# pangenome/sweepga

Measured on AMD Instinct MI355X. Metric: PAF mappings/sec through plane-sweep+scaffold filter, 1/2/4/8 MI355X, higher is better.
Workload: dtype u32 coordinates, f64 scores; 1 GPU; BASELINE.json configs[3] (synthetic 100 M mappings across 10 k (q,t) groups, 100-genome pangenome shape; S-pan in SURVEY.md 8d): 100000000 mappings per GPU over 9900 genome-pair groups (100 single-chromosome genomes), pipeline=default; flags=(defaults), mappings_per_gpu=100000000, groups_per_gpu=9900

## Files before the change

sweepga_amd/csrc/swg_chain_table.hip:

```cpp
#include "swg_scaffold_internal.h"

namespace swg_scaf {
namespace {

__global__ __launch_bounds__(EW) void seg_compose_kernel(uint64_t m, const uint32_t* __restrict__ s_gidx,
                                                         const uint32_t* __restrict__ v, int complement,
                                                         uint64_t* __restrict__ out) {
  uint64_t p = (uint64_t)blockIdx.x * EW + threadIdx.x;
  if (p < m) out[p] = ((uint64_t)s_gidx[p] << 32) | (complement ? 0xffffffffu - v[p] : v[p]);
}
__global__ __launch_bounds__(EW) void group_first_from_scan_kernel(uint64_t m, const uint32_t* __restrict__ head_flag,
                                                                   const uint64_t* __restrict__ run_max,
                                                                   uint32_t* __restrict__ group_first) {
  uint64_t p = (uint64_t)blockIdx.x * EW + threadIdx.x;
  if (p >= m) return;
  if (p + 1 == m || head_flag[p + 1]) {
    const uint64_t v = run_max[p];
    group_first[(uint32_t)(v >> 32)] = 0xffffffffu - (uint32_t)v;
  }
}

constexpr int HEAD_SPAN = 1024;
__global__ __launch_bounds__(EW) void head_init_kernel(uint64_t m, const uint32_t* __restrict__ pred,
                                                       uint32_t* __restrict__ hd, const uint8_t* __restrict__ only,
// ... 212 lines not shown
        if (*slot > vmin) atomicMin(slot, vmin);
      }
    } else {
#pragma unroll
      for (int u = 0; u < U; ++u)
        if (live[u]) {
          uint32_t* slot = pair_slot(table, (uint32_t)(L[u] >> 32), (uint32_t)L[u]);
          if (*slot > (uint32_t)(i0 + u)) atomicMin(slot, (uint32_t)(i0 + u));
        }
    }
  }
}

__global__ __launch_bounds__(EW) void genome_pair_first_groups_kernel(uint32_t n_groups, const uint32_t* __restrict__ group_begin,
                                                                      const uint32_t* __restrict__ s_idx,
                                                                      const uint32_t* __restrict__ group_first,
                                                                      const uint32_t* __restrict__ q_id,
                                                                      const uint32_t* __restrict__ t_id,
                                                                      const uint32_t* __restrict__ seq_genome, PairTable table) {
  uint32_t g = blockIdx.x * EW + threadIdx.x;
  if (g >= n_groups) return;
  const uint32_t i = s_idx[group_begin[g]];
  atomicMin(pair_slot(table, seq_genome[q_id[i]], seq_genome[t_id[i]]), group_first[g]);
}

__device__ __forceinline__ uint32_t heads_before(const uint32_t* __restrict__ ch_head, uint32_t nc, uint32_t p) {
  uint32_t l = 0, r = nc;
  while (l < r) {
    const uint32_t mid = l + ((r - l) >> 1);
    if (ch_head[mid] < p)
      l = mid + 1;
    else
      r = mid;
  }
  return l;
}
__global__ __launch_bounds__(EW) void group_keys_kernel(uint32_t n_groups, const uint32_t* __restrict__ group_begin,
                                                        uint32_t m, const uint32_t* __restrict__ ch_head, uint32_t nc,
                                                        const uint32_t* __restrict__ s_idx,
                                                        const uint32_t* __restrict__ group_first,
                                                        const uint32_t* __restrict__ q_id,
                                                        const uint32_t* __restrict__ t_id,
                                                        const uint32_t* __restrict__ seq_genome, bool pair_major,
                                                        PairTable gp_first, int idx_bits,
                                                        uint64_t* __restrict__ g_key, uint32_t* __restrict__ g_val,
                                                        uint32_t* __restrict__ g_first_chain,
                                                        uint32_t* __restrict__ g_nchains) {
  uint32_t g = blockIdx.x * EW + threadIdx.x;
  if (g >= n_groups) return;
  const uint32_t b = group_begin[g];
  const uint32_t first = heads_before(ch_head, nc, b);
  const uint32_t next = (g + 1 < n_groups) ? heads_before(ch_head, nc, group_begin[g + 1]) : nc;
  (void)m;
  g_first_chain[g] = first;
  g_nchains[g] = next - first;
  const uint32_t i = s_idx[b];
  uint64_t hi = 0;
  if (pair_major) hi = pair_get(gp_first, seq_genome[q_id[i]], seq_genome[t_id[i]]);
  g_key[g] = (hi << idx_bits) | group_first[g];
  g_val[g] = g;
}
__global__ __launch_bounds__(EW) void group_sizes_sorted_kernel(uint32_t n_groups, const uint32_t* __restrict__ g_sorted,
                                                                const uint32_t* __restrict__ g_nchains,
                                                                uint32_t* __restrict__ sizes) {
  uint32_t r = blockIdx.x * EW + threadIdx.x;
  if (r < n_groups) sizes[r] = g_nchains[g_sorted[r]];
}
__global__ __launch_bounds__(EW) void group_base_kernel(uint32_t n_groups, const uint32_t* __restrict__ g_sorted,
                                                        const uint32_t* __restrict__ base_sorted,
                                                        uint32_t* __restrict__ g_base) {
  uint32_t r = blockIdx.x * EW + threadIdx.x;
  if (r < n_groups) g_base[g_sorted[r]] = base_sorted[r];
}
__global__ __launch_bounds__(EW) void chain_place_kernel(uint64_t nc, const uint32_t* __restrict__ ch_head,
                                                         const uint32_t* __restrict__ s_gidx,
                                                         const uint32_t* __restrict__ g_first_chain,
                                                         const uint32_t* __restrict__ g_base, uint32_t* __restrict__ order) {
  uint64_t c = (uint64_t)blockIdx.x * EW + threadIdx.x;
  if (c >= nc) return;
  const uint32_t g = s_gidx[ch_head[c]];
  order[g_base[g] + ((uint32_t)c - g_first_chain[g])] = (uint32_t)c;
}

__global__ __launch_bounds__(EW) void chain_ok_kernel(uint64_t m, const uint32_t* __restrict__ is_head,
                                                      const uint32_t* __restrict__ s_qs, const uint32_t* __restrict__ h_qe,
                                                      const uint32_t* __restrict__ h_ts, const uint32_t* __restrict__ h_te,
                                                      const unsigned long long* __restrict__ h_sm,
                                                      const unsigned long long* __restrict__ h_sb,
                                                      const uint64_t* __restrict__ s_grp, uint64_t min_len,
                                                      double min_ident, uint8_t* __restrict__ ok_head,
                                                      HeadRec* __restrict__ rec, const uint8_t* __restrict__ only,
                                                      const uint8_t* __restrict__ span) {
  const uint64_t n_span = (m + HEAD_SPAN - 1) / HEAD_SPAN;
  for (uint64_t sp = blockIdx.x; sp < n_span; sp += gridDim.x) {
    if (span && !span[sp]) continue;
    for (int k = threadIdx.x; k < HEAD_SPAN; k += EW) {
      const uint64_t p = sp * HEAD_SPAN + k;
      if (p >= m) break;
      if (only && !only[p]) continue;
      bool ok = false;
      if (is_head[p] != 0) {
        const uint64_t total_length = (uint64_t)h_qe[p] - (uint64_t)s_qs[p];
        ok = total_length >= min_len;
        if (ok) {
          const double wid = chain_weighted_identity(total_length, h_sm[p], h_sb[p]);
          ok = wid >= min_ident;
          if (ok) {
            HeadRec hr;
            hr.qs = s_qs[p];
            hr.qe = h_qe[p];
            hr.ts = h_ts[p];
            hr.te = h_te[p];
            hr.wid = wid;
            hr.grp = s_grp[p];
            rec[p] = hr;
          }
        }
      }
      ok_head[p] = ok ? 1 : 0;
    }
  }
}

constexpr int LABEL_CAP = (int)(WALK_CHUNK + BIG_UNIT);
constexpr int LABEL_FAST = (int)LABEL_FAST_ELEMS;
constexpr int LABEL_NT = 512;
static_assert(LABEL_FAST * (2 + 2 + 3 * 4) >= LABEL_CAP * 2, "the two layouts share one LDS buffer");
template <int NT, bool MB, bool RANKED>
__global__ __launch_bounds__(NT, RANKED ? 8 : 1) void chain_label_kernel(uint32_t n_chunks, const SpecBlock* __restrict__ chunks,
                                                         const uint32_t* __restrict__ pred,
                                                         const uint32_t* __restrict__ s_qs, const uint32_t* __restrict__ s_qe,
                                                         const uint32_t* __restrict__ s_ts, const uint32_t* __restrict__ s_te,
                                                         const uint32_t* __restrict__ s_m, const uint32_t* __restrict__ s_b,
                                                         const uint64_t* __restrict__ s_grp,
                                                         uint64_t min_len, double min_ident, uint32_t* __restrict__ hd,
                                                         uint8_t* __restrict__ ok_head, HeadRec* __restrict__ rec,
                                                         unsigned long long* __restrict__ n_heads,
                                                         const uint32_t* __restrict__ n_chunks_dev = nullptr, LabelRanked R = LabelRanked{}) {
  if (n_chunks_dev) n_chunks = min(n_chunks, *n_chunks_dev);
  __shared__ uint32_t lds[LABEL_FAST * (MB ? 6 : 4)];
  uint16_t* succ = reinterpret_cast<uint16_t*>(lds);
  uint16_t* l_hd = succ + LABEL_FAST;
  uint32_t* l_qe = lds + LABEL_FAST;
  uint32_t* l_ts = l_qe + LABEL_FAST;
  uint32_t* l_te = l_ts + LABEL_FAST;
  uint32_t* l_m = MB ? l_te + LABEL_FAST : nullptr;
  uint32_t* l_b = MB ? l_m + LABEL_FAST : nullptr;
  __shared__ uint64_t ws64[RANKED ? NT / 64 : 1];
  if (!MB) s_m = s_b = nullptr;
  constexpr uint16_t NO = 0xffffu;
  uint32_t heads = 0;
  for (uint32_t c = blockIdx.x; c < n_chunks; c += gridDim.x) {
    const uint32_t b = chunks[c].bb, e = chunks[c].be;
    uint32_t len = e > b ? e - b : 0;
    if (len >= (uint32_t)LABEL_CAP) len = 0;
    __syncthreads();
    for (uint32_t k = threadIdx.x; k < len; k += NT) succ[k] = NO;
    __syncthreads();
    if (len <= (uint32_t)LABEL_FAST) {
      constexpr int U = LABEL_FAST / NT;
      static_assert(LABEL_FAST % NT == 0, "whole rounds");
      uint32_t r_pr[U], r_qe[U], r_ts[U], r_te[U], r_m[U], r_b[U], r_qs[U];
#pragma unroll
      for (int u = 0; u < U; ++u) {
        const uint32_t k = (uint32_t)u * NT + threadIdx.x;
        const uint32_t p = b + (k < len ? k : 0u);
        r_pr[u] = pred[p];
        r_qe[u] = s_qe[p];
        r_ts[u] = s_ts[p];
        r_te[u] = s_te[p];
        r_m[u] = s_m ? s_m[p] : 0u;
        r_b[u] = s_m ? s_b[p] : 0u;
        r_qs[u] = s_qs[p];
      }
#pragma unroll
      for (int u = 0; u < U; ++u) {
        const uint32_t k = (uint32_t)u * NT + threadIdx.x;
        if (k < len) {
          if (r_pr[u] != NONE) succ[r_pr[u] - b] = (uint16_t)k;
          l_hd[k] = r_pr[u] != NONE ? NO : (uint16_t)k;
          l_qe[k] = r_qe[u];
          l_ts[k] = r_ts[u];
          l_te[k] = r_te[u];
          if constexpr (MB) {
            l_m[k] = r_m[u];
            l_b[k] = r_b[u];
          }
        }
      }
      __syncthreads();
      const uint32_t pad = RANKED ? chunks[c].pad : 0u;
      const bool rkd = RANKED && (pad & CHUNK_RANKED) != 0u;
      uint32_t pass = 0;
#pragma unroll
      for (int u = 0; u < U; ++u) {
        const uint32_t k = (uint32_t)u * NT + threadIdx.x;
        if (k >= len) continue;
        const uint32_t p = b + k;
        if (r_pr[u] != NONE) {
          if (!rkd) ok_head[p] = 0;
          continue;
        }
        ++heads;
        uint32_t qe = r_qe[u], ts = r_ts[u], te = r_te[u];
        uint64_t sm = r_m[u], sb = r_b[u];
        for (uint16_t nx = succ[k]; nx != NO; nx = succ[nx]) {
          const uint32_t a = l_qe[nx], t0 = l_ts[nx], t1 = l_te[nx];
          l_hd[nx] = (uint16_t)k;
          qe = a > qe ? a : qe;
          ts = t0 < ts ? t0 : ts;
          te = t1 > te ? t1 : te;
          if constexpr (MB) {
            sm += l_m[nx];
            sb += l_b[nx];
          }
        }
        const uint32_t qs0 = r_qs[u];
        const uint64_t total_length = (uint64_t)qe - (uint64_t)qs0;
        bool ok = total_length >= min_len;
        if (ok) {
          const double wid = chain_weighted_identity(total_length, sm, sb);
          ok = wid >= min_ident;
          if (ok && !rkd) {
            HeadRec hr;
            hr.qs = qs0;
            hr.qe = qe;
            hr.ts = ts;
            hr.te = te;
            hr.wid = wid;
            hr.grp = s_grp ? s_grp[p] : 0ull;
            rec[p] = hr;
          }
        }
        if (rkd) {
          if (ok) {
            pass |= 1u << u;
            l_qe[k] = qe;
            l_ts[k] = ts;
            l_te[k] = qs0;
            if (!(qs0 < qe && ts < te)) atomicOr(R.flags, R.fallback_bit);
          } else {
            succ[k] = NO;
          }
          continue;
        }
        ok_head[p] = ok ? (uint8_t)(s_grp ? 1u : 1u | (qs0 < qe ? 2u : 0u) | (ts < te ? 4u : 0u)) : (uint8_t)0;
      }
      if constexpr (RANKED) {
        if (rkd) {
          uint64_t packed = 0;
#pragma unroll
          for (int u = 0; u < U; ++u) packed |= (uint64_t)((pass >> u) & 1u) << (16 * u);
          static_assert(U <= 4 && NT < 65536, "the rows' counters share a 64-bit word");
          uint64_t inc = packed;
          const int lane = threadIdx.x & 63, w = threadIdx.x >> 6;
#pragma unroll
          for (int d = 1; d < 64; d <<= 1) {
            const uint64_t t = __shfl_up(inc, d, 64);
            if (lane >= d) inc += t;
          }
          if (lane == 63) ws64[w] = inc;
          __syncthreads();
          uint64_t off = 0, tot = 0;
#pragma unroll
          for (int j = 0; j < NT / 64; ++j) {
            const uint64_t x = ws64[j];
            off += j < w ? x : 0ull;
            tot += x;
          }
          const uint64_t ex = off + inc - packed;
          uint32_t row_base = 0;
#pragma unroll
          for (int u = 0; u < U; ++u) {
            const uint32_t k = (uint32_t)u * NT + threadIdx.x;
            if ((pass >> u) & 1u) {
              const uint32_t r = row_base + (uint32_t)((ex >> (16 * u)) & 0xffffu);
              succ[k] = (uint16_t)r;
              if ((pad & 1u) == 0u) {
                R.t_qs[b + r] = l_te[k];
                R.t_qe[b + r] = l_qe[k];
                reinterpret_cast<uint32_t*>(rec + b)[r] = l_ts[k];
              }
            }
            row_base += (uint32_t)((tot >> (16 * u)) & 0xffffu);
          }
          if (threadIdx.x == 0) R.chunk_pass[c] = row_base;
          __syncthreads();
          for (uint32_t k = threadIdx.x; k < len; k += NT) {
            const uint16_t r = succ[l_hd[k]];
            hd[b + k] = r == NO ? NONE : (uint32_t)r;
          }
          continue;
        }
      }
      __syncthreads();
      for (uint32_t k = threadIdx.x; k < len; k += NT) hd[b + k] = b + l_hd[k];
      continue;
    }
    constexpr int LB = 2048 / NT;
    for (uint32_t k0 = 0; k0 < len; k0 += NT * LB) {
      uint32_t pr[LB];
#pragma unroll
      for (int u = 0; u < LB; ++u) {
        const uint32_t k = k0 + (uint32_t)u * NT + threadIdx.x;
        pr[u] = pred[b + (k < len ? k : 0u)];
      }
#pragma unroll
      for (int u = 0; u < LB; ++u) {
        const uint32_t k = k0 + (uint32_t)u * NT + threadIdx.x;
        if (k < len && pr[u] != NONE) succ[pr[u] - b] = (uint16_t)k;
      }
    }
    __syncthreads();
    for (uint32_t k0 = 0; k0 < len; k0 += NT * LB) {
      uint32_t pr[LB], v_qs[LB], v_qe[LB], v_ts[LB], v_te[LB], v_m[LB], v_b[LB];
#pragma unroll
      for (int u = 0; u < LB; ++u) {
        const uint32_t k = k0 + (uint32_t)u * NT + threadIdx.x;
        const uint32_t p = b + (k < len ? k : 0u);
        pr[u] = pred[p];
        v_qs[u] = s_qs[p];
        v_qe[u] = s_qe[p];
        v_ts[u] = s_ts[p];
        v_te[u] = s_te[p];
        v_m[u] = s_m ? s_m[p] : 0u;
        v_b[u] = s_m ? s_b[p] : 0u;
      }
#pragma unroll
      for (int u = 0; u < LB; ++u) {
        const uint32_t k = k0 + (uint32_t)u * NT + threadIdx.x;
        if (k >= len) continue;
        const uint32_t p = b + k;
        if (pr[u] != NONE) {
          ok_head[p] = 0;
          continue;
        }
        ++heads;
        hd[p] = p;
        uint32_t qe = v_qe[u], ts = v_ts[u], te = v_te[u];
        uint64_t sm = v_m[u], sb = v_b[u];
        for (uint16_t nx = succ[k]; nx != NO;) {
          const uint32_t q = b + nx;
          const uint16_t nn = succ[nx];
          const uint32_t a = s_qe[q], t0 = s_ts[q], t1 = s_te[q], mm = s_m ? s_m[q] : 0u, bb = s_m ? s_b[q] : 0u;
          hd[q] = p;
          qe = a > qe ? a : qe;
          ts = t0 < ts ? t0 : ts;
          te = t1 > te ? t1 : te;
          sm += mm;
          sb += bb;
          nx = nn;
        }
        const uint32_t qs0 = v_qs[u];
        const uint64_t total_length = (uint64_t)qe - (uint64_t)qs0;
        bool ok = total_length >= min_len;
        if (ok) {
          const double wid = chain_weighted_identity(total_length, sm, sb);
          ok = wid >= min_ident;
          if (ok) {
            HeadRec hr;
            hr.qs = qs0;
            hr.qe = qe;
            hr.ts = ts;
            hr.te = te;
            hr.wid = wid;
            hr.grp = s_grp ? s_grp[p] : 0ull;
            rec[p] = hr;
          }
        }
        ok_head[p] = ok ? (uint8_t)(s_grp ? 1u : 1u | (qs0 < qe ? 2u : 0u) | (ts < te ? 4u : 0u)) : (uint8_t)0;
      }
    }
  }
#pragma unroll
  for (int o = 32; o > 0; o >>= 1) heads += __shfl_down(heads, o, 64);
  __syncthreads();
  if ((threadIdx.x & 63) == 0) lds[threadIdx.x >> 6] = heads;
  __syncthreads();
  if (threadIdx.x == 0) {
    uint32_t all = 0;
    for (int w = 0; w < NT / 64; ++w) all += lds[w];
    if (all) atomicAdd(n_heads, (unsigned long long)all);
  }
}
__global__ __launch_bounds__(1024) void chain_label_long_kernel(uint32_t cap_long, const uint32_t* __restrict__ n_long_dev,
                                                                const uint32_t* __restrict__ long_list,
                                                                const SpecBlock* __restrict__ chunks, const uint32_t* __restrict__ pred,
                                                                const uint32_t* __restrict__ s_qs, const uint32_t* __restrict__ s_qe,
                                                                const uint32_t* __restrict__ s_ts, const uint32_t* __restrict__ s_te,
                                                                const uint32_t* __restrict__ s_m, const uint32_t* __restrict__ s_b,
                                                                uint64_t min_len, double min_ident, uint32_t* hd,
                                                                uint8_t* __restrict__ ok_head, HeadRec* rec,
                                                                unsigned long long* __restrict__ n_heads) {
// ... 341 lines not shown
```

sweepga_amd/csrc/swg_pair.hip:

```cpp
#include <cmath>
#include <type_traits>

#include "swg_scaffold_internal.h"

namespace swg_scaf {
namespace {

constexpr uint32_t PAIR_CELL = WALK_CHUNK;
constexpr uint32_t PAIR_S_MAX = 1024, PAIR_M_MAX = 4096, PAIR_L_MAX = 32768, PAIR_XL_MAX = uint32_t(1) << 18;
constexpr uint32_t PAIR_XL_CELLS = PAIR_XL_MAX / PAIR_CELL;
constexpr uint32_t PAIR_HASH_MAX = 65536;
constexpr uint32_t PAIR_MX_MAX = 16384, PAIR_MX_CUT_DEFAULT = 8192;
constexpr uint32_t ORDER_BIN_L = 128;
constexpr uint32_t ORDERED = 0x80000000u;
constexpr uint32_t PF_NOT_GROUPED = 1, PF_RUN_OVERFLOW = 2, PF_TOO_LONG = 4, PF_FALLBACK = 8;

struct PairRun {
  uint32_t a, n;
};
struct PairInfo {
  uint32_t m;
  uint32_t m_plus;
  uint32_t M;
  uint32_t first_alive;
// ... 1536 lines not shown
  uint8_t* status;
  uint32_t* chain;
  int scaffolds_only;
  uint64_t gap;
  uint64_t max_dev;
  uint64_t rescue_d;
  uint64_t max_s2;
  const uint8_t* kept_in;
  const uint32_t* chain_base;
  const uint32_t* np;
  const SpecBlock* chunks;
  uint32_t cap_chunks;
  const uint32_t* chunk_pass;
  uint32_t* rec_w;
  unsigned long long* ranked_stat;
  uint32_t* fin;
  uint32_t* anum;
  uint32_t* n_out_pair;
  PairCounters* C;
};
constexpr uint32_t NEVER = 0xfffffffeu;

struct PairChainArgs {
  const PairRun* runs;
  const uint32_t* list;
  const uint32_t* list_xl;
  uint32_t n_xl;
  const PairInfo* info;
  const uint8_t* ok_head;
  const HeadRec* rec;
  uint32_t *T_qs, *T_qe, *T_ts, *T_te;
  double* T_wid;
  uint64_t* T_seg;
  uint32_t *chain_base, *np;
  uint32_t *cnt, *has, *stretch;
  PairRun* T_runs;
  unsigned long long* totals;
  const PairCounters* C;
};
template <int NT, int PHASE>
__global__ __launch_bounds__(NT) void pair_chains_kernel(PairChainArgs A) {
  constexpr int U = 4;
  __shared__ uint32_t ws[NT / 64 + 1];
  __shared__ uint64_t ws64[NT / 64 + 1];
  __shared__ uint32_t sh_base;
  const int tid = threadIdx.x;
  if (A.C->flags & PF_FALLBACK) return;
  const uint32_t rk = blockIdx.x < A.n_xl ? A.list_xl[blockIdx.x] : A.list[blockIdx.x - A.n_xl];
  const PairRun run = A.runs[rk];
  const PairInfo pi = A.info[rk];
  const uint32_t a = run.a, m = pi.m, m_plus = pi.m_plus;
  if (PHASE == 0) {
    uint32_t c0 = 0, c1 = 0, mx = 0;
    for (uint32_t p0 = 0; p0 < m; p0 += NT * U) {
      uint8_t ok[U];
#pragma unroll
      for (int u = 0; u < U; ++u) {
        const uint32_t p = p0 + (uint32_t)u * NT + (uint32_t)tid;
        ok[u] = p < m ? A.ok_head[a + p] : (uint8_t)0;
      }
#pragma unroll
      for (int u = 0; u < U; ++u) {
        const uint32_t p = p0 + (uint32_t)u * NT + (uint32_t)tid;
        if (ok[u]) {
          const HeadRec hr = A.rec[a + p];
          if (p < m_plus) ++c0; else ++c1;
          const uint32_t e = hr.qe > hr.te ? hr.qe : hr.te;
          mx = e > mx ? e : mx;
        }
      }
    }
    const uint32_t nP = block_sum<NT>(c0, ws), nM = block_sum<NT>(c1, ws);
#pragma unroll
    for (int o = 32; o > 0; o >>= 1) {
      const uint32_t t = __shfl_xor(mx, o, 64);
      mx = t > mx ? t : mx;
    }
    if ((tid & 63) == 0 && (unsigned long long)mx > __hip_atomic_load(&A.totals[1], __ATOMIC_RELAXED, __HIP_MEMORY_SCOPE_AGENT))
      atomicMax(&A.totals[1], (unsigned long long)mx);
    if (tid == 0) {
      A.np[2 * rk] = nP;
      A.np[2 * rk + 1] = nM;
      A.cnt[rk] = nP + nM;
      A.has[rk] = nP + nM ? 1u : 0u;
    }
    return;
  }
  const uint32_t nP = A.np[2 * rk], nM = A.np[2 * rk + 1];
  if (nP + nM == 0) return;
  const uint32_t cb = A.chain_base[rk];
  if (tid == 0) {
    PairRun tr;
    tr.a = cb;
    tr.n = nP + nM;
    A.T_runs[A.stretch[rk]] = tr;
  }
  (void)sh_base;
  const bool plus_first = pi.first_mem[0] < pi.first_mem[1];
  uint32_t before = 0;
  for (uint32_t p0 = 0; p0 < m; p0 += NT * U) {
    uint8_t ok[U];
    uint64_t packed = 0;
#pragma unroll
    for (int u = 0; u < U; ++u) {
      const uint32_t p = p0 + (uint32_t)u * NT + (uint32_t)tid;
      ok[u] = p < m ? A.ok_head[a + p] : (uint8_t)0;
      packed |= (uint64_t)(ok[u] ? 1u : 0u) << (16 * u);
    }
    uint64_t inc = packed;
    const int lane = tid & 63, w = tid >> 6;
#pragma unroll
    for (int d = 1; d < 64; d <<= 1) {
      const uint64_t t = __shfl_up(inc, d, 64);
      if (lane >= d) inc += t;
    }
    uint64_t off = 0, tot = 0;
    if (NT == 64) {
      tot = __shfl(inc, 63, 64);
    } else {
      __syncthreads();
      if (lane == 63) ws64[w] = inc;
      __syncthreads();
#pragma unroll
      for (int k = 0; k < NT / 64; ++k) {
        const uint64_t x = ws64[k];
        off += k < w ? x : 0ull;
        tot += x;
      }
    }
    const uint64_t ex = off + inc - packed;
    uint32_t row_base = before;
#pragma unroll
    for (int u = 0; u < U; ++u) {
      const uint32_t p = p0 + (uint32_t)u * NT + (uint32_t)tid;
      if (ok[u]) {
        const uint32_t c_pos = row_base + (uint32_t)((ex >> (16 * u)) & 0xffffu);
        const uint32_t c_all = plus_first ? c_pos : (p >= m_plus ? c_pos - nP : c_pos + nM);
        const HeadRec hr = A.rec[a + p];
        const uint32_t c = cb + c_all;
        A.T_qs[c] = hr.qs;
        A.T_qe[c] = hr.qe;
        A.T_ts[c] = hr.ts;
        A.T_te[c] = hr.te;
        A.T_wid[c] = hr.wid;
        A.T_seg[c] = rk;
      }
      row_base += (uint32_t)((tot >> (16 * u)) & 0xffffu);
    }
    before = row_base;
  }
}

template <int NT, int KP>
__global__ __launch_bounds__(NT, NT >= 512 ? 4 : 1) void pair_finish_kernel(PairFinishArgs A) {
  constexpr int U = 4;
  __shared__ uint32_t ws[NT / 64 + 1];
  __shared__ uint64_t ws64[NT / 64 + 1];
  __shared__ uint64_t ws64n[2 * (NT / 64 + 1)];
  __shared__ uint32_t l_all[4 * KP];
  uint32_t* const l_qs = l_all;
  uint32_t* const l_qe = l_all + KP;
  uint32_t* const l_ts = l_all + 2 * KP;
  uint32_t* const l_pm = l_all + 3 * KP;
  const int tid = threadIdx.x;
#ifdef SWG_PAIR_TIMING
  unsigned long long pt_last = wall_clock64();
#endif
  if (A.C->flags & PF_FALLBACK) return;
  const uint32_t rk = blockIdx.x < A.n_xl ? A.list_xl[blockIdx.x] : A.list[blockIdx.x - A.n_xl];
  const PairRun run = A.runs[rk];
  const PairInfo pi = A.info[rk];
  const uint32_t a = run.a, m = pi.m, m_plus = pi.m_plus, M = pi.M;
  PairSum sm;
  sm.n_pass = sm.n_kept = 0;
  sm.minmem = NONE;
  sm.base = 0;
  if (m == 0) {
    if (tid == 0) A.sum[rk] = sm;
    return;
  }
  uint32_t n_pass0 = 0, n_pass1 = 0, n_q = 0, n_deg = 0, n_kept = 0, kP = 0;
  bool all_q = false, all_t = false;
  const bool given = A.kept_in != nullptr;
  const uint32_t g_nP = given ? A.np[2 * rk] : 0u, g_nM = given ? A.np[2 * rk + 1] : 0u, g_cb = given ? A.chain_base[rk] : 0u;
  const bool plus_first0 = pi.first_mem[0] < pi.first_mem[1];
  auto row_scan = [&](uint64_t packed, uint64_t* tot_out) -> uint64_t {
    uint64_t inc = packed;
    const int lane = tid & 63, w = tid >> 6;
#pragma unroll
    for (int d = 1; d < 64; d <<= 1) {
      const uint64_t t = __shfl_up(inc, d, 64);
      if (lane >= d) inc += t;
    }
    uint64_t off = 0, tot = 0;
    if (NT == 64) {
      tot = __shfl(inc, 63, 64);
    } else {
      lds_barrier();
      if (lane == 63) ws64[w] = inc;
      lds_barrier();
#pragma unroll
      for (int k = 0; k < NT / 64; ++k) {
        const uint64_t x = ws64[k];
        off += k < w ? x : 0ull;
        tot += x;
      }
    }
    *tot_out = tot;
    return off + inc - packed;
  };
  auto row_scan_n = [&](auto g_c, const uint64_t (&packed)[decltype(g_c)::value], uint64_t (&ex)[decltype(g_c)::value],
                        uint64_t (&tot)[decltype(g_c)::value]) {
    constexpr int G = decltype(g_c)::value;
    uint64_t inc[G];
    const int lane = tid & 63, w = tid >> 6;
#pragma unroll
    for (int g = 0; g < G; ++g) inc[g] = packed[g];
#pragma unroll
    for (int d = 1; d < 64; d <<= 1) {
#pragma unroll
      for (int g = 0; g < G; ++g) {
        const uint64_t t = __shfl_up(inc[g], d, 64);
        if (lane >= d) inc[g] += t;
      }
    }
    if (NT == 64) {
#pragma unroll
      for (int g = 0; g < G; ++g) {
        tot[g] = __shfl(inc[g], 63, 64);
        ex[g] = inc[g] - packed[g];
      }
      return;
    }
    lds_barrier();
    if (lane == 63) {
#pragma unroll
      for (int g = 0; g < G; ++g) ws64n[g * (NT / 64 + 1) + w] = inc[g];
    }
    lds_barrier();
#pragma unroll
    for (int g = 0; g < G; ++g) {
      uint64_t off = 0, t = 0;
#pragma unroll
      for (int k = 0; k < NT / 64; ++k) {
        const uint64_t x = ws64n[g * (NT / 64 + 1) + k];
        off += k < w ? x : 0ull;
        t += x;
      }
      tot[g] = t;
      ex[g] = off + inc[g] - packed[g];
    }
  };
  constexpr int US = NT >= 512 ? 8 : 4;
  constexpr int GS = US / 4;
  auto sweep = [&](const bool exact) {
    uint32_t kept_before = 0, ok_before = 0, c0 = 0, c1 = 0, cq = 0, cd = 0, cp = 0;
    for (uint32_t p0 = 0; p0 < m; p0 += NT * US) {
      uint8_t ok[US];
      uint32_t h_qs[US], h_qe[US], h_ts[US];
#pragma unroll
      for (int u = 0; u < US; ++u) {
        const uint32_t p = p0 + (uint32_t)u * NT + (uint32_t)tid;
        ok[u] = p < m ? A.ok_head[a + p] : (uint8_t)0;
      }
      bool kept[US];
      if (given) {
        uint64_t okp[GS], ex_ok[GS], tot_ok[GS];
#pragma unroll
        for (int g = 0; g < GS; ++g) okp[g] = 0;
#pragma unroll
        for (int u = 0; u < US; ++u) okp[u / 4] |= (uint64_t)(ok[u] ? 1u : 0u) << (16 * (u % 4));
        row_scan_n(std::integral_constant<int, GS>{}, okp, ex_ok, tot_ok);
        uint32_t rb = ok_before;
#pragma unroll
        for (int u = 0; u < US; ++u) {
          const uint32_t p = p0 + (uint32_t)u * NT + (uint32_t)tid;
          kept[u] = false;
          if (ok[u]) {
            const uint32_t c_pos = rb + (uint32_t)((ex_ok[u / 4] >> (16 * (u % 4))) & 0xffffu);
            const uint32_t c_all = plus_first0 ? c_pos : (p >= m_plus ? c_pos - g_nP : c_pos + g_nM);
            kept[u] = A.kept_in[g_cb + c_all] != 0;
          }
          rb += (uint32_t)((tot_ok[u / 4] >> (16 * (u % 4))) & 0xffffu);
        }
        ok_before = rb;
      }
      uint64_t packed[GS], ex[GS], tot[GS];
#pragma unroll
      for (int g = 0; g < GS; ++g) packed[g] = 0;
#pragma unroll
      for (int u = 0; u < US; ++u) {
        const uint32_t p = p0 + (uint32_t)u * NT + (uint32_t)tid;
        if (!given) kept[u] = false;
        if (ok[u]) {
          const bool hq = (ok[u] & 2u) != 0, ht = (ok[u] & 4u) != 0;
          if (!given) kept[u] = exact ? (all_q || hq) && (all_t || ht) : hq && ht;
          if (p < m_plus) ++c0; else ++c1;
          cq += hq ? 1u : 0u;
          cd += (given || (hq && ht)) ? 0u : 1u;
          cp += (kept[u] && p < m_plus) ? 1u : 0u;
        }
        packed[u / 4] |= (uint64_t)(kept[u] ? 1u : 0u) << (16 * (u % 4));
      }
#pragma unroll
      for (int u = 0; u < US; ++u) {
        const uint32_t p = p0 + (uint32_t)u * NT + (uint32_t)tid;
        h_qs[u] = h_qe[u] = h_ts[u] = 0;
        if (kept[u] && p < m_plus) {
          const HeadRec* hp = A.rec + a + p;
          h_qs[u] = hp->qs;
          h_qe[u] = hp->qe;
          h_ts[u] = hp->ts;
        }
      }
      row_scan_n(std::integral_constant<int, GS>{}, packed, ex, tot);
      uint32_t row_base = kept_before;
#pragma unroll
      for (int u = 0; u < US; ++u) {
        const uint32_t p = p0 + (uint32_t)u * NT + (uint32_t)tid;
        const uint32_t r = row_base + (uint32_t)((ex[u / 4] >> (16 * (u % 4))) & 0xffffu);
        if (p < m) A.head_num[a + p] = kept[u] ? r : (ok[u] ? NEVER : NONE);
        if (kept[u] && p < m_plus) {
          A.f_qs[a + r] = h_qs[u];
          A.f_qe[a + r] = h_qe[u];
          A.f_ts[a + r] = h_ts[u];
          if (r < (uint32_t)KP) {
            l_qs[r] = h_qs[u];
            l_qe[r] = h_qe[u];
            l_ts[r] = h_ts[u];
          }
        }
        row_base += (uint32_t)((tot[u / 4] >> (16 * (u % 4))) & 0xffffu);
      }
      kept_before = row_base;
    }
    n_kept = kept_before;
    n_pass0 = block_sum<NT>(c0, ws);
    n_pass1 = block_sum<NT>(c1, ws);
    n_q = block_sum<NT>(cq, ws);
    n_deg = block_sum<NT>(cd, ws);
    kP = block_sum<NT>(cp, ws);
  };
  const bool plus_first = plus_first0;
  uint32_t kM = 0, out = 0;
  auto local_number = [&](uint32_t r, bool minus) -> uint32_t {
    if (plus_first) return r + 1;
    return minus ? r - kP + 1 : r + kM + 1;
  };
  const uint32_t slot0 = A.chunks ? a / PAIR_CELL + 2u * rk : 0u;
  const bool ranked = A.chunks && slot0 < A.cap_chunks && (A.chunks[slot0].pad & CHUNK_RANKED) != 0u;
  if (ranked) {
    __shared__ uint32_t rk_beg[RANKED_MAX_CHUNKS], rk_base[RANKED_MAX_CHUNKS + 1], rk_n[3];
    if (A.ranked_stat && tid == 0) {
      atomicAdd(&A.ranked_stat[0], 1ull);
      atomicAdd(&A.ranked_stat[1], (unsigned long long)run.n);
    }
    if (tid < 64) {
      uint32_t lim = run.n / PAIR_CELL + 2u;
      lim = lim < RANKED_MAX_CHUNKS ? lim : RANKED_MAX_CHUNKS;
      lim = lim < A.cap_chunks - slot0 ? lim : A.cap_chunks - slot0;
      uint32_t carry = 0, nck = 0, kp = 0;
      for (uint32_t j0 = 0; j0 < lim; j0 += 64) {
        const uint32_t j = j0 + (uint32_t)tid;
        SpecBlock d;
        d.ue = d.bb = d.be = d.pad = 0u;
        if (j < lim) d = A.chunks[slot0 + j];
        const bool valid = d.be > d.bb;
        const uint32_t cnt = valid ? A.chunk_pass[slot0 + j] : 0u;
        uint32_t inc = cnt;
#pragma unroll
        for (int dd = 1; dd < 64; dd <<= 1) {
          const uint32_t t = __shfl_up(inc, dd, 64);
          if (tid >= dd) inc += t;
        }
        if (valid) {
          rk_beg[j] = d.bb - a;
          rk_base[j] = carry + inc - cnt;
        }
        kp += valid && (d.pad & 1u) == 0u ? cnt : 0u;
        nck += (uint32_t)__popcll(__ballot(valid));
        carry += __shfl(inc, 63, 64);
      }
#pragma unroll
      for (int o = 32; o > 0; o >>= 1) kp += __shfl_xor(kp, o, 64);
      if (tid == 0) {
        rk_base[nck] = carry;
        rk_n[0] = nck;
        rk_n[1] = kp;
        rk_n[2] = carry;
      }
    }
    __syncthreads();
    const uint32_t nck = rk_n[0];
    kP = rk_n[1];
    n_kept = rk_n[2];
    kM = n_kept - kP;
    if (n_kept == 0) {
      if (tid == 0) A.sum[rk] = sm;
      return;
    }
    sm.n_pass = n_kept;
    sm.n_kept = n_kept;
    sm.minmem = kP && kM ? (pi.first_mem[0] < pi.first_mem[1] ? pi.first_mem[0] : pi.first_mem[1]) : (kP ? pi.first_mem[0] : pi.first_mem[1]);
    if (tid == 0) A.sum[rk] = sm;
    FT_STAMP(0);
    uint32_t cj = 0, c_base = rk_base[0], c_next = nck > 1u ? rk_beg[1] : NONE;
    for (uint32_t p0 = 0; p0 < m; p0 += NT * US) {
      uint32_t r[US];
#pragma unroll
      for (int u = 0; u < US; ++u) {
        const uint32_t p = p0 + (uint32_t)u * NT + (uint32_t)tid;
        r[u] = p < m ? A.hd[a + p] : NONE;
      }
#pragma unroll
      for (int u = 0; u < US; ++u) {
        const uint32_t p = p0 + (uint32_t)u * NT + (uint32_t)tid;
        if (p >= m) continue;
        while (p >= c_next) {
          ++cj;
          c_base = rk_base[cj];
          c_next = cj + 1u < nck ? rk_beg[cj + 1u] : NONE;
        }
        uint32_t f = 0u;
        if (r[u] != NONE) {
          f = ((uint32_t)SWG_ST_SCAFFOLD << 30) | local_number(c_base + r[u], p >= m_plus);
          ++out;
        }
        A.fin[a + p] = f;
      }
    }
    for (uint32_t p = m + (uint32_t)tid; p < M; p += NT) A.fin[a + p] = 0u;
    if (!A.scaffolds_only && kP > 0 && M > m_plus) {
      const bool in_lds = kP <= (uint32_t)KP;
      uint32_t *const g_qs = A.f_qs + a, *const g_qe = A.f_qe + a, *const g_ts = A.rec_w + (size_t)8 * a;
      for (uint32_t c0 = 0; c0 < kP; c0 += NT) {
        const uint32_t c = c0 + (uint32_t)tid;
        uint32_t v_qs = 0, v_qe = 0, v_ts = 0;
        if (c < kP) {
          uint32_t lo = 0, hi = nck;
          while (hi - lo > 1u) {
            const uint32_t mid = (lo + hi) >> 1;
            if (rk_base[mid] <= c) lo = mid; else hi = mid;
          }
          const uint32_t b = rk_beg[lo], i = c - rk_base[lo];
          v_qs = A.f_qs[a + b + i];
          v_qe = A.f_qe[a + b + i];
          v_ts = A.rec_w[(size_t)8 * (a + b) + i];
        }
        if (in_lds) {
          if (c < kP) {
            l_qs[c] = v_qs;
            l_qe[c] = v_qe;
            l_ts[c] = v_ts;
          }
        } else {
          __syncthreads();
          if (c < kP) {
            g_qs[c] = v_qs;
            g_qe[c] = v_qe;
            g_ts[c] = v_ts;
          }
        }
      }
      __syncthreads();
    }
  } else {
    sweep(false);
    const uint32_t n_ch = n_pass0 + n_pass1;
    if (n_ch == 0) {
      if (tid == 0) A.sum[rk] = sm;
      return;
    }
    if (n_deg) {
      all_q = n_ch <= 1;
      all_t = (all_q ? n_ch : n_q) <= 1;
      __syncthreads();
      sweep(true);
    }
    kM = n_kept - kP;
    sm.n_pass = n_ch;
    sm.n_kept = n_kept;
    sm.minmem = n_pass0 && n_pass1 ? (pi.first_mem[0] < pi.first_mem[1] ? pi.first_mem[0] : pi.first_mem[1]) : (n_pass0 ? pi.first_mem[0] : pi.first_mem[1]);
    if (tid == 0) A.sum[rk] = sm;
    if (n_kept == 0) return;
    __syncthreads();
    FT_STAMP(0);
    for (uint32_t p0 = 0; p0 < m; p0 += NT * US) {
      uint32_t h[US], idx[US], r[US];
#pragma unroll
      for (int u = 0; u < US; ++u) {
        const uint32_t p = p0 + (uint32_t)u * NT + (uint32_t)tid;
        h[u] = p < m ? A.hd[a + p] : a;
        idx[u] = (p < m && !A.fin) ? A.s_idx[a + p] : 0u;
      }
#pragma unroll
      for (int u = 0; u < US; ++u) r[u] = A.head_num[h[u]];
#pragma unroll
      for (int u = 0; u < US; ++u) {
        const uint32_t p = p0 + (uint32_t)u * NT + (uint32_t)tid;
        uint32_t an = 0;
        if (p < m && r[u] < NEVER) {
          an = local_number(r[u], h[u] - a >= m_plus);
          if (!A.fin) {
            A.chain[idx[u]] = an;
            A.status[idx[u]] = SWG_ST_SCAFFOLD;
          }
          ++out;
        } else if (r[u] == NEVER) {
          an = NEVER;
        }
        if (A.fin && p < m) A.fin[a + p] = (an != 0u && an != NEVER) ? ((uint32_t)SWG_ST_SCAFFOLD << 30) | an : 0u;
        if (A.rescue_d && p < m) A.anum[a + p] = an;
      }
    }
    for (uint32_t p = m + (uint32_t)tid; p < M; p += NT) {
      if (A.rescue_d) A.anum[a + p] = 0u;
      if (A.fin) A.fin[a + p] = 0u;
    }
  }
  FT_STAMP(1);
  if (!A.scaffolds_only && kP > 0 && M > m_plus) {
    const bool in_lds = kP <= (uint32_t)KP;
    uint32_t *const g_qs = A.f_qs + a, *const g_qe = A.f_qe + a;
    uint32_t* const g_ts = ranked ? A.rec_w + (size_t)8 * a : A.f_ts + a;
    uint32_t* const g_pm = ranked ? g_ts + m : A.f_pm + a;
    uint64_t carry = 0;
    for (uint32_t c0b = 0; c0b < kP; c0b += NT) {
      const uint32_t c = c0b + tid;
      const uint64_t v = c < kP ? (uint64_t)(in_lds ? l_qe[c] : g_qe[c]) : 0ull;
      uint64_t tot;
      uint64_t ex = block_excl_max<NT>(v, ws64, &tot);
      ex = ex > carry ? ex : carry;
      if (c < kP) {
        const uint32_t pm = (uint32_t)(v > ex ? v : ex);
        if (in_lds) l_pm[c] = pm; else g_pm[c] = pm;
      }
      carry = tot > carry ? tot : carry;
    }
    __syncthreads();
    const uint32_t* __restrict__ c_qs = in_lds ? l_qs : g_qs;
    const uint32_t* __restrict__ c_qe = in_lds ? l_qe : g_qe;
    const uint32_t* __restrict__ c_ts = in_lds ? l_ts : g_ts;
    const uint32_t* __restrict__ c_pm = in_lds ? l_pm : g_pm;
    const uint64_t gap = A.gap, max_dev = A.max_dev;
    for (uint32_t p = m_plus + tid; p < M; p += NT) {
      const uint32_t iw = A.s_idx[a + p];
      if (p >= m && (iw >> 31) == 0) continue;
      const uint32_t i = iw & 0x7fffffffu;
      const uint64_t qs = A.s_qs[a + p], qe = A.s_qe[a + p], ts = A.s_ts[a + p], te = A.s_te[a + p];
      if (A.fin ? A.fin[a + p] != 0u : A.chain[i] != 0u) continue;
      const uint64_t qc = (qs + qe) / 2, tc = (ts + te) / 2;
      const uint64_t lim = qe > ~0ull - gap ? ~0ull : qe + gap;
      uint32_t l = 0, r = kP;
      while (l < r) {
        const uint32_t mid = l + ((r - l) >> 1);
        if ((uint64_t)c_qs[mid] <= lim) l = mid + 1; else r = mid;
      }
      uint32_t lo = 0, hi = l;
      while (lo < hi) {
        const uint32_t mid = lo + ((hi - lo) >> 1);
        const uint64_t pm = c_pm[mid];
        if ((pm > ~0ull - gap ? ~0ull : pm + gap) < qs) lo = mid + 1; else hi = mid;
      }
      uint32_t best = NONE;
      for (uint32_t c = lo; c < l; ++c) {
        const uint64_t cqe = c_qe[c];
        if ((cqe > ~0ull - gap ? ~0ull : cqe + gap) < qs) continue;
        const int64_t diag = (int64_t)c_ts[c] - (int64_t)c_qs[c];
        const int64_t dev = (int64_t)tc - (int64_t)qc - diag;
        const uint64_t deviation = dev < 0 ? (uint64_t)0 - (uint64_t)dev : (uint64_t)dev;
        if (deviation <= max_dev) {
          best = c;
          break;
        }
      }
      if (best != NONE) {
        const uint32_t num = local_number(best, false);
        if (A.fin) {
          A.fin[a + p] = ((uint32_t)SWG_ST_SCAFFOLD << 30) | num;
        } else {
          A.chain[i] = num;
          A.status[i] = SWG_ST_SCAFFOLD;
        }
        if (A.rescue_d) A.anum[a + p] = num;
        ++out;
      }
    }
  }
  FT_STAMP(2);
  if (!A.scaffolds_only && A.rescue_d) {
    __syncthreads();
    const uint64_t D = A.rescue_d, max_s2 = A.max_s2;
    int cell_sh = 0;
    while (cell_sh < 32 && (1ull << cell_sh) <= D) ++cell_sh;
    constexpr uint32_t NB = (uint32_t)KP / 2u, KA = (4u * (uint32_t)KP - NB - 1u) / 3u, BT = NB / NT;
    static_assert(KA >= (uint32_t)NT * U && KA < 65536u && NB % (2 * NT) == 0, "one round of anchors fits a batch; whole words of bins per thread");
    uint32_t* const g_qc = l_all;
    uint32_t* const g_tc = l_all + KA;
    uint32_t* const g_ix = l_all + 2 * KA;
    uint16_t* const b_start = reinterpret_cast<uint16_t*>(l_all + 3 * KA);
    uint32_t* const b_cur = l_all + 3 * KA + (NB + 2) / 2;
    auto bump = [&](uint32_t b) -> uint32_t {
      const uint32_t sh = 16u * (b & 1u);
      return (atomicAdd(&b_cur[b >> 1], 1u << sh) >> sh) & 0xffffu;
    };
    uint32_t* const c_num = A.f_qe + a;
    auto is_anchor = [](uint32_t an) { return an != 0u && an < 0x80000000u; };
    static_assert((NB & (NB - 1u)) == 0u && NB >= 4u, "bins by the cell's low bits");
    auto cell_of = [&](uint32_t qc) -> uint32_t { return cell_sh < 32 ? qc >> cell_sh : 0u; };
    auto bin_of = [&](uint32_t qc) -> uint32_t { return cell_of(qc) & (NB - 1u); };
    uint32_t pb = 0, r0 = 0;
    while (pb < M) {
      for (uint32_t b = tid; b < NB / 2; b += NT) b_cur[b] = 0u;
      __syncthreads();
      uint32_t cnt = 0, pe = pb;
      for (uint32_t p0 = pb; p0 < M; p0 += NT * U) {
        uint32_t an[U], qs[U], qe[U];
#pragma unroll
        for (int u = 0; u < U; ++u) {
          const uint32_t p = p0 + (uint32_t)u * NT + (uint32_t)tid;
          const uint32_t j = a + (p < M ? p : 0u);
          an[u] = p < M ? A.anum[j] : 0u;
          qs[u] = A.s_qs[j];
          qe[u] = A.s_qe[j];
        }
        uint32_t mine = 0;
#pragma unroll
        for (int u = 0; u < U; ++u) mine += is_anchor(an[u]) ? 1u : 0u;
        const uint32_t rt = block_sum<NT>(mine, ws);
        if (cnt + rt > KA) break;
#pragma unroll
        for (int u = 0; u < U; ++u)
          if (is_anchor(an[u])) (void)bump(bin_of((uint32_t)(((uint64_t)qs[u] + qe[u]) / 2)));
        cnt += rt;
        pe = p0 + NT * U < M ? p0 + NT * U : M;
      }
      __syncthreads();
      {
        uint32_t c[BT], sum = 0;
#pragma unroll
        for (uint32_t k = 0; k < BT; k += 2) {
          const uint32_t w = b_cur[((uint32_t)tid * BT + k) >> 1];
          c[k] = w & 0xffffu;
          c[k + 1] = w >> 16;
          sum += c[k] + c[k + 1];
        }
        uint32_t tot;
        uint32_t run = block_excl_sum<NT>(sum, ws, &tot);
#pragma unroll
        for (uint32_t k = 0; k < BT; k += 2) {
          const uint32_t s0 = run, s1 = run + c[k];
          b_start[(uint32_t)tid * BT + k] = (uint16_t)s0;
          b_start[(uint32_t)tid * BT + k + 1] = (uint16_t)s1;
          b_cur[((uint32_t)tid * BT + k) >> 1] = s0 | (s1 << 16);
          run = s1 + c[k + 1];
        }
        if (tid == NT - 1) b_start[NB] = (uint16_t)run;
      }
      __syncthreads();
      for (uint32_t p0 = pb; p0 < pe; p0 += NT * U) {
        uint32_t an[U], qs[U], qe[U], ts[U], te[U], ix[U];
#pragma unroll
        for (int u = 0; u < U; ++u) {
          const uint32_t p = p0 + (uint32_t)u * NT + (uint32_t)tid;
          const uint32_t j = a + (p < pe ? p : 0u);
          an[u] = p < pe ? A.anum[j] : 0u;
          qs[u] = A.s_qs[j];
          qe[u] = A.s_qe[j];
          ts[u] = A.s_ts[j];
          te[u] = A.s_te[j];
          ix[u] = A.s_idx[j];
        }
#pragma unroll
        for (int u = 0; u < U; ++u) {
          if (!is_anchor(an[u])) continue;
          const uint32_t qc = (uint32_t)(((uint64_t)qs[u] + qe[u]) / 2);
          const uint32_t e = bump(bin_of(qc));
          g_qc[e] = qc;
          g_tc[e] = (uint32_t)(((uint64_t)ts[u] + te[u]) / 2);
          g_ix[e] = ix[u] & 0x7fffffffu;
          c_num[r0 + e] = an[u];
        }
      }
      __syncthreads();
      FT_STAMP(3);
      for (uint32_t p0 = 0; cnt && p0 < M; p0 += NT * U) {
        uint32_t an[U], qs[U], qe[U], ts[U], te[U];
#pragma unroll
        for (int u = 0; u < U; ++u) {
          const uint32_t p = p0 + (uint32_t)u * NT + (uint32_t)tid;
          const uint32_t j = a + (p < M ? p : 0u);
          an[u] = A.anum[j];
          qs[u] = A.s_qs[j];
          qe[u] = A.s_qe[j];
          ts[u] = A.s_ts[j];
          te[u] = A.s_te[j];
        }
#pragma unroll
        for (int u = 0; u < U; ++u) {
          const uint32_t p = p0 + (uint32_t)u * NT + (uint32_t)tid;
          const uint32_t st = an[u];
          if (p >= M || !(st == 0u || (st >= 0x80000000u && st != NEVER))) continue;
          const uint32_t qc32 = (uint32_t)(((uint64_t)qs[u] + qe[u]) / 2);
// ... 916 lines not shown
```

Before: 14.29 billion mappings/s.

## Prefetch ranked-chunk metadata and anchor heads, skip unused te loads in ranked labeling

In the label kernel, ranked chunks no longer load or accumulate target-end values, which were never used on that path, and the fallback check drops the ts<te test. In pair_finish, the ranked-chunk table and the first round of head words are loaded before the branch, and head words are software-prefetched one round ahead. Anchor inputs in the rescue loop are also prefetched one iteration ahead, and fin/chain lookups are replaced by a head-word check. A 7-waves occupancy hint is added for 256-thread blocks, and the fallback early return becomes a zero-work path that keeps the barrier structure uniform. These changes trade more live registers and some speculative loads for shorter memory latency chains.

```diff
diff --git a/sweepga_amd/csrc/swg_chain_table.hip b/sweepga_amd/csrc/swg_chain_table.hip
--- a/sweepga_amd/csrc/swg_chain_table.hip
+++ b/sweepga_amd/csrc/swg_chain_table.hip
@@ -388,6 +388,8 @@
   uint32_t heads = 0;
   for (uint32_t c = blockIdx.x; c < n_chunks; c += gridDim.x) {
     const uint32_t b = chunks[c].bb, e = chunks[c].be;
+    const uint32_t pad = RANKED ? chunks[c].pad : 0u;
+    const bool rkd = RANKED && (pad & CHUNK_RANKED) != 0u;
     uint32_t len = e > b ? e - b : 0;
     if (len >= (uint32_t)LABEL_CAP) len = 0;
     __syncthreads();
@@ -404,7 +406,7 @@
         r_pr[u] = pred[p];
         r_qe[u] = s_qe[p];
         r_ts[u] = s_ts[p];
-        r_te[u] = s_te[p];
+        r_te[u] = rkd ? 0u : s_te[p];
         r_m[u] = s_m ? s_m[p] : 0u;
         r_b[u] = s_m ? s_b[p] : 0u;
         r_qs[u] = s_qs[p];
@@ -417,7 +419,7 @@
           l_hd[k] = r_pr[u] != NONE ? NO : (uint16_t)k;
           l_qe[k] = r_qe[u];
           l_ts[k] = r_ts[u];
-          l_te[k] = r_te[u];
+          if (!rkd) l_te[k] = r_te[u];
           if constexpr (MB) {
             l_m[k] = r_m[u];
             l_b[k] = r_b[u];
@@ -425,8 +427,6 @@
         }
       }
       __syncthreads();
-      const uint32_t pad = RANKED ? chunks[c].pad : 0u;
-      const bool rkd = RANKED && (pad & CHUNK_RANKED) != 0u;
       uint32_t pass = 0;
 #pragma unroll
       for (int u = 0; u < U; ++u) {
@@ -440,15 +440,28 @@
         ++heads;
         uint32_t qe = r_qe[u], ts = r_ts[u], te = r_te[u];
         uint64_t sm = r_m[u], sb = r_b[u];
-        for (uint16_t nx = succ[k]; nx != NO; nx = succ[nx]) {
-          const uint32_t a = l_qe[nx], t0 = l_ts[nx], t1 = l_te[nx];
-          l_hd[nx] = (uint16_t)k;
-          qe = a > qe ? a : qe;
-          ts = t0 < ts ? t0 : ts;
-          te = t1 > te ? t1 : te;
-          if constexpr (MB) {
-            sm += l_m[nx];
-            sb += l_b[nx];
+        if (rkd) {
+          for (uint16_t nx = succ[k]; nx != NO; nx = succ[nx]) {
+            const uint32_t a = l_qe[nx], t0 = l_ts[nx];
+            l_hd[nx] = (uint16_t)k;
+            qe = a > qe ? a : qe;
+            ts = t0 < ts ? t0 : ts;
+            if constexpr (MB) {
+              sm += l_m[nx];
+              sb += l_b[nx];
+            }
+          }
+        } else {
+          for (uint16_t nx = succ[k]; nx != NO; nx = succ[nx]) {
+            const uint32_t a = l_qe[nx], t0 = l_ts[nx], t1 = l_te[nx];
+            l_hd[nx] = (uint16_t)k;
+            qe = a > qe ? a : qe;
+            ts = t0 < ts ? t0 : ts;
+            te = t1 > te ? t1 : te;
+            if constexpr (MB) {
+              sm += l_m[nx];
+              sb += l_b[nx];
+            }
           }
         }
         const uint32_t qs0 = r_qs[u];
@@ -474,7 +487,7 @@
             l_qe[k] = qe;
             l_ts[k] = ts;
             l_te[k] = qs0;
-            if (!(qs0 < qe && ts < te)) atomicOr(R.flags, R.fallback_bit);
+            if (!(qs0 < qe)) atomicOr(R.flags, R.fallback_bit);
           } else {
             succ[k] = NO;
           }
diff --git a/sweepga_amd/csrc/swg_pair.hip b/sweepga_amd/csrc/swg_pair.hip
--- a/sweepga_amd/csrc/swg_pair.hip
+++ b/sweepga_amd/csrc/swg_pair.hip
@@ -1712,7 +1712,7 @@
 }
 
 template <int NT, int KP>
-__global__ __launch_bounds__(NT, NT >= 512 ? 4 : 1) void pair_finish_kernel(PairFinishArgs A) {
+__global__ __launch_bounds__(NT, NT >= 512 ? 4 : NT >= 256 ? 7 : 1) void pair_finish_kernel(PairFinishArgs A) {
   constexpr int U = 4;
   __shared__ uint32_t ws[NT / 64 + 1];
   __shared__ uint64_t ws64[NT / 64 + 1];
@@ -1726,17 +1726,18 @@
 #ifdef SWG_PAIR_TIMING
   unsigned long long pt_last = wall_clock64();
 #endif
-  if (A.C->flags & PF_FALLBACK) return;
+  const uint32_t call_flags = A.C->flags;
   const uint32_t rk = blockIdx.x < A.n_xl ? A.list_xl[blockIdx.x] : A.list[blockIdx.x - A.n_xl];
   const PairRun run = A.runs[rk];
   const PairInfo pi = A.info[rk];
-  const uint32_t a = run.a, m = pi.m, m_plus = pi.m_plus, M = pi.M;
+  const bool gave_up = (call_flags & PF_FALLBACK) != 0u;
+  const uint32_t a = run.a, m = gave_up ? 0u : pi.m, m_plus = pi.m_plus, M = pi.M;
   PairSum sm;
   sm.n_pass = sm.n_kept = 0;
   sm.minmem = NONE;
   sm.base = 0;
   if (m == 0) {
-    if (tid == 0) A.sum[rk] = sm;
+    if (tid == 0 && !gave_up) A.sum[rk] = sm;
     return;
   }
   uint32_t n_pass0 = 0, n_pass1 = 0, n_q = 0, n_deg = 0, n_kept = 0, kP = 0;
@@ -1908,50 +1909,77 @@
     return minus ? r - kP + 1 : r + kM + 1;
   };
   const uint32_t slot0 = A.chunks ? a / PAIR_CELL + 2u * rk : 0u;
-  const bool ranked = A.chunks && slot0 < A.cap_chunks && (A.chunks[slot0].pad & CHUNK_RANKED) != 0u;
+  __shared__ uint32_t rk_beg[RANKED_MAX_CHUNKS], rk_base[RANKED_MAX_CHUNKS + 1], rk_n[3];
+  uint32_t lim = 0, cnt0 = 0, nck = 0;
+  SpecBlock d0;
+  d0.ue = d0.bb = d0.be = d0.pad = 0u;
+  uint32_t hd_nx[US];
+#pragma unroll
+  for (int u = 0; u < US; ++u) hd_nx[u] = NONE;
+  if (A.chunks) {
+    if (tid < 64 && slot0 < A.cap_chunks) {
+      lim = run.n / PAIR_CELL + 2u;
+      lim = lim < RANKED_MAX_CHUNKS ? lim : RANKED_MAX_CHUNKS;
+      lim = lim < A.cap_chunks - slot0 ? lim : A.cap_chunks - slot0;
+      const uint32_t j = (uint32_t)tid < lim ? (uint32_t)tid : 0u;
+      d0 = A.chunks[slot0 + j];
+      cnt0 = A.chunk_pass[slot0 + j];
+    }
+#pragma unroll
+    for (int u = 0; u < US; ++u) {
+      const uint32_t p = (uint32_t)u * NT + (uint32_t)tid;
+      hd_nx[u] = A.hd[a + (p < m ? p : 0u)];
+    }
+    if (tid < 64) {
+      const bool mark = (__shfl(d0.pad, 0, 64) & CHUNK_RANKED) != 0u;
+      uint32_t carry = 0, nc = 0, kp = 0;
+      for (uint32_t j0 = 0; mark && j0 < lim; j0 += 64) {
+        const uint32_t j = j0 + (uint32_t)tid;
+        SpecBlock d = d0;
+        uint32_t cnt = cnt0;
+        if (j0) {
+          d.ue = d.bb = d.be = d.pad = 0u;
+          cnt = 0u;
+          if (j < lim) {
+            d = A.chunks[slot0 + j];
+            cnt = A.chunk_pass[slot0 + j];
+          }
+        }
+        const bool valid = j < lim && d.be > d.bb;
+        cnt = valid ? cnt : 0u;
+        uint32_t inc = cnt;
+#pragma unroll
+        for (int dd = 1; dd < 64; dd <<= 1) {
+          const uint32_t t = __shfl_up(inc, dd, 64);
+          if (tid >= dd) inc += t;
+        }
+        if (valid) {
+          rk_beg[j] = d.bb - a;
+          rk_base[j] = carry + inc - cnt;
+        }
+        kp += valid && (d.pad & 1u) == 0u ? cnt : 0u;
+        nc += (uint32_t)__popcll(__ballot(valid));
+        carry += __shfl(inc, 63, 64);
+      }
+#pragma unroll
+      for (int o = 32; o > 0; o >>= 1) kp += __shfl_xor(kp, o, 64);
+      if (tid == 0) {
+        rk_base[nc] = carry;
+        rk_n[0] = nc | (mark ? 0x80000000u : 0u);
+        rk_n[1] = kp;
+        rk_n[2] = carry;
+      }
+    }
+    lds_barrier();
+    nck = rk_n[0];
+  }
+  const bool ranked = (nck >> 31) != 0u;
+  nck &= 0x7fffffffu;
   if (ranked) {
-    __shared__ uint32_t rk_beg[RANKED_MAX_CHUNKS], rk_base[RANKED_MAX_CHUNKS + 1], rk_n[3];
     if (A.ranked_stat && tid == 0) {
       atomicAdd(&A.ranked_stat[0], 1ull);
       atomicAdd(&A.ranked_stat[1], (unsigned long long)run.n);
     }
-    if (tid < 64) {
-      uint32_t lim = run.n / PAIR_CELL + 2u;
-      lim = lim < RANKED_MAX_CHUNKS ? lim : RANKED_MAX_CHUNKS;
-      lim = lim < A.cap_chunks - slot0 ? lim : A.cap_chunks - slot0;
-      uint32_t carry = 0, nck = 0, kp = 0;
-      for (uint32_t j0 = 0; j0 < lim; j0 += 64) {
-        const uint32_t j = j0 + (uint32_t)tid;
-        SpecBlock d;
-        d.ue = d.bb = d.be = d.pad = 0u;
-        if (j < lim) d = A.chunks[slot0 + j];
-        const bool valid = d.be > d.bb;
-        const uint32_t cnt = valid ? A.chunk_pass[slot0 + j] : 0u;
-        uint32_t inc = cnt;
-#pragma unroll
-        for (int dd = 1; dd < 64; dd <<= 1) {
-          const uint32_t t = __shfl_up(inc, dd, 64);
-          if (tid >= dd) inc += t;
-        }
-        if (valid) {
-          rk_beg[j] = d.bb - a;
-          rk_base[j] = carry + inc - cnt;
-        }
-        kp += valid && (d.pad & 1u) == 0u ? cnt : 0u;
-        nck += (uint32_t)__popcll(__ballot(valid));
-        carry += __shfl(inc, 63, 64);
-      }
-#pragma unroll
-      for (int o = 32; o > 0; o >>= 1) kp += __shfl_xor(kp, o, 64);
-      if (tid == 0) {
-        rk_base[nck] = carry;
-        rk_n[0] = nck;
-        rk_n[1] = kp;
-        rk_n[2] = carry;
-      }
-    }
-    __syncthreads();
-    const uint32_t nck = rk_n[0];
     kP = rk_n[1];
     n_kept = rk_n[2];
     kM = n_kept - kP;
@@ -1965,17 +1993,22 @@
     if (tid == 0) A.sum[rk] = sm;
     FT_STAMP(0);
     uint32_t cj = 0, c_base = rk_base[0], c_next = nck > 1u ? rk_beg[1] : NONE;
-    for (uint32_t p0 = 0; p0 < m; p0 += NT * US) {
+    auto anchors_round = [&](const uint32_t p0, auto whole_c) {
+      constexpr bool WHOLE = decltype(whole_c)::value;
       uint32_t r[US];
+#pragma unroll
+      for (int u = 0; u < US; ++u) r[u] = hd_nx[u];
+      if (WHOLE) {
+#pragma unroll
+        for (int u = 0; u < US; ++u) {
+          const uint32_t p = p0 + NT * US + (uint32_t)u * NT + (uint32_t)tid;
+          hd_nx[u] = A.hd[a + (p < m ? p : 0u)];
+        }
+      }
 #pragma unroll
       for (int u = 0; u < US; ++u) {
         const uint32_t p = p0 + (uint32_t)u * NT + (uint32_t)tid;
-        r[u] = p < m ? A.hd[a + p] : NONE;
-      }
-#pragma unroll
-      for (int u = 0; u < US; ++u) {
-        const uint32_t p = p0 + (uint32_t)u * NT + (uint32_t)tid;
-        if (p >= m) continue;
+        if (!WHOLE && p >= m) continue;
         while (p >= c_next) {
           ++cj;
           c_base = rk_base[cj];
@@ -1988,32 +2021,49 @@
         }
         A.fin[a + p] = f;
       }
-    }
+    };
+    uint32_t p0 = 0;
+    for (; p0 + NT * US <= m; p0 += NT * US) anchors_round(p0, std::true_type{});
+    if (p0 < m) anchors_round(p0, std::false_type{});
     for (uint32_t p = m + (uint32_t)tid; p < M; p += NT) A.fin[a + p] = 0u;
     if (!A.scaffolds_only && kP > 0 && M > m_plus) {
-      const bool in_lds = kP <= (uint32_t)KP;
-      uint32_t *const g_qs = A.f_qs + a, *const g_qe = A.f_qe + a, *const g_ts = A.rec_w + (size_t)8 * a;
-      for (uint32_t c0 = 0; c0 < kP; c0 += NT) {
-        const uint32_t c = c0 + (uint32_t)tid;
-        uint32_t v_qs = 0, v_qe = 0, v_ts = 0;
-        if (c < kP) {
-          uint32_t lo = 0, hi = nck;
-          while (hi - lo > 1u) {
-            const uint32_t mid = (lo + hi) >> 1;
-            if (rk_base[mid] <= c) lo = mid; else hi = mid;
+      auto triple_at = [&](uint32_t c, uint32_t& v_qs, uint32_t& v_qe, uint32_t& v_ts) {
+        uint32_t lo = 0, hi = nck;
+        while (hi - lo > 1u) {
+          const uint32_t mid = (lo + hi) >> 1;
+          if (rk_base[mid] <= c) lo = mid; else hi = mid;
+        }
+        const uint32_t b = rk_beg[lo], i = c - rk_base[lo];
+        v_qs = A.f_qs[a + b + i];
+        v_qe = A.f_qe[a + b + i];
+        v_ts = A.rec_w[(size_t)8 * (a + b) + i];
+      };
+      if (kP <= (uint32_t)KP) {
+        constexpr int RT = 2;
+        for (uint32_t c0 = 0; c0 < kP; c0 += RT * NT) {
+          uint32_t v_qs[RT], v_qe[RT], v_ts[RT];
+#pragma unroll
+          for (int k = 0; k < RT; ++k) {
+            const uint32_t c = c0 + (uint32_t)k * NT + (uint32_t)tid;
+            v_qs[k] = v_qe[k] = v_ts[k] = 0u;
+            if (c < kP) triple_at(c, v_qs[k], v_qe[k], v_ts[k]);
           }
-          const uint32_t b = rk_beg[lo], i = c - rk_base[lo];
-          v_qs = A.f_qs[a + b + i];
-          v_qe = A.f_qe[a + b + i];
-          v_ts = A.rec_w[(size_t)8 * (a + b) + i];
-        }
-        if (in_lds) {
-          if (c < kP) {
-            l_qs[c] = v_qs;
-            l_qe[c] = v_qe;
-            l_ts[c] = v_ts;
+#pragma unroll
+          for (int k = 0; k < RT; ++k) {
+            const uint32_t c = c0 + (uint32_t)k * NT + (uint32_t)tid;
+            if (c < kP) {
+              l_qs[c] = v_qs[k];
+              l_qe[c] = v_qe[k];
+              l_ts[c] = v_ts[k];
+            }
           }
-        } else {
+        }
+      } else {
+        uint32_t *const g_qs = A.f_qs + a, *const g_qe = A.f_qe + a, *const g_ts = A.rec_w + (size_t)8 * a;
+        for (uint32_t c0 = 0; c0 < kP; c0 += NT) {
+          const uint32_t c = c0 + (uint32_t)tid;
+          uint32_t v_qs = 0, v_qe = 0, v_ts = 0;
+          if (c < kP) triple_at(c, v_qs, v_qe, v_ts);
           __syncthreads();
           if (c < kP) {
             g_qs[c] = v_qs;
@@ -2103,12 +2153,38 @@
     const uint32_t* __restrict__ c_ts = in_lds ? l_ts : g_ts;
     const uint32_t* __restrict__ c_pm = in_lds ? l_pm : g_pm;
     const uint64_t gap = A.gap, max_dev = A.max_dev;
+    uint32_t n_iw = 0, n_qs = 0, n_qe = 0, n_ts = 0, n_te = 0, n_hd = NONE;
+    if (ranked) {
+      const uint32_t pc = m_plus + (uint32_t)tid < M ? m_plus + (uint32_t)tid : 0u;
+      n_iw = A.s_idx[a + pc];
+      n_qs = A.s_qs[a + pc];
+      n_qe = A.s_qe[a + pc];
+      n_ts = A.s_ts[a + pc];
+      n_te = A.s_te[a + pc];
+      n_hd = A.hd[a + (pc < m ? pc : 0u)];
+    }
     for (uint32_t p = m_plus + tid; p < M; p += NT) {
-      const uint32_t iw = A.s_idx[a + p];
-      if (p >= m && (iw >> 31) == 0) continue;
+      uint32_t iw;
+      uint64_t qs, qe, ts, te;
+      if (ranked) {
+        iw = n_iw;
+        qs = n_qs, qe = n_qe, ts = n_ts, te = n_te;
+        const uint32_t hdw = n_hd, pn = p + NT < M ? p + NT : 0u;
+        n_iw = A.s_idx[a + pn];
+        n_qs = A.s_qs[a + pn];
+        n_qe = A.s_qe[a + pn];
+        n_ts = A.s_ts[a + pn];
+        n_te = A.s_te[a + pn];
+        n_hd = A.hd[a + (pn < m ? pn : 0u)];
+        if (p >= m && (iw >> 31) == 0) continue;
+        if (p < m && hdw != NONE) continue;
+      } else {
+        iw = A.s_idx[a + p];
+        if (p >= m && (iw >> 31) == 0) continue;
+        qs = A.s_qs[a + p], qe = A.s_qe[a + p], ts = A.s_ts[a + p], te = A.s_te[a + p];
+        if (A.fin ? A.fin[a + p] != 0u : A.chain[iw & 0x7fffffffu] != 0u) continue;
+      }
       const uint32_t i = iw & 0x7fffffffu;
-      const uint64_t qs = A.s_qs[a + p], qe = A.s_qe[a + p], ts = A.s_ts[a + p], te = A.s_te[a + p];
-      if (A.fin ? A.fin[a + p] != 0u : A.chain[i] != 0u) continue;
       const uint64_t qc = (qs + qe) / 2, tc = (ts + te) / 2;
       const uint64_t lim = qe > ~0ull - gap ? ~0ull : qe + gap;
       uint32_t l = 0, r = kP;
```

Result: faster. 14.47 billion mappings/s, median of 6 (+1.3%).
